# GuoYi0/alphaFive

Hardware: AMD Instinct MI355X
Metric: self-play moves/sec (11x11, 500 sims/move) (higher is better)
Workload: dtype f32 (fp16x2 split operands: 3 fp16 MFMA products per MAC, fp32 accumulate)

## Files before the change

alphafive_amd/csrc/af_engine.hip:

```cpp

#include <hip/hip_runtime.h>
#include <stdint.h>
#include <stdio.h>
#include <stdlib.h>
#include <string.h>

#include <type_traits>
#include <vector>

#include "af_engine.h"
#include "af_noise.h"

typedef unsigned long long u64;

enum { PH_IDLE = 0, PH_MOVE_START = 1, PH_SEARCH = 2, PH_MOVE_DONE = 3, PH_ERROR = 4, PH_DESCENT = 5  };
enum { CT_SIMS = 0, CT_SELECTS, CT_EXPANDS, CT_TERMINALS, CT_PLIES, CT_EPISODES, CT_LSUM, CT_LEXP,
       CT_GC, CT_GC_SCANNED, CT_YIELDS, CT_STALLS, CT_N };
enum { HIST_WORK = 0, HIST_TIME = 64, HIST_MAXTIME = 96, HIST_N = 97 };

struct EngineParams {
    int G, S, C, goal, sims, upper, training, mode, node_cap, max_ply, budget, budget_hard;
    uint32_t hash_mask;
    double init_temp, tau_decay, tau_decay_r, alpha, c_puct;
    float c_puct32;
// ... 3 lines not shown
    int32_t *action, *has_policy, *visits;
    float* policy;
    u64 *root, *leaf;
    double* tau;
    uint32_t *episode, *sel, *plyctr;
    int32_t *path_node, *path_cell;
    uint32_t* hash;
    u64* node_key;
    int32_t* node_sum;
    int32_t* free_idx;
    int32_t* edge_n;
    float *edge_w, *edge_p;
    int32_t* edge_c;
    double* edge_w64;
    int32_t w64;
    uint32_t *ep_seq, *ep_popped;
    int32_t* ep_len;
    float* ep_final;
    u64* rec_key;
    float* rec_policy;
    int32_t *rec_visits, *rec_last, *rec_action;
    u64* counters;
    u64* progress;
    u64* hist;
    u64* memo_key;
    float* memo_pv;
    float* memo_val;
    u64* memo_lock;
    u64* memo_stats;
    uint32_t memo_bucket_mask;
    int memo_max_stones;
    uint32_t memo_epoch;
    int memo_budget;
};
enum { MEMO_SERIAL = 0, MEMO_PROBES, MEMO_HITS, MEMO_INSERTS, MEMO_REPLACED, MEMO_N };

__device__ __forceinline__ uint32_t rfl32(uint32_t x) { return (uint32_t)__builtin_amdgcn_readfirstlane((int)x); }
__device__ __forceinline__ int rfli(int x) { return __builtin_amdgcn_readfirstlane(x); }
__device__ __forceinline__ u64 rfl64(u64 x) {
    return ((u64)rfl32((uint32_t)(x >> 32)) << 32) | (u64)rfl32((uint32_t)x);
}
__device__ __forceinline__ float rflf(float x) { return __int_as_float(rfli(__float_as_int(x))); }
template <int CTRL, int ROWS = 0xF>
__device__ __forceinline__ int dpp_i(int v) { return __builtin_amdgcn_update_dpp(v, v, CTRL, ROWS, 0xF, false); }
__device__ __forceinline__ int wave_max_i32(int v) {
    int o;
    o = dpp_i<0xB1>(v); v = o > v ? o : v;
    o = dpp_i<0x4E>(v); v = o > v ? o : v;
    o = dpp_i<0x141>(v); v = o > v ? o : v;
    o = dpp_i<0x140>(v); v = o > v ? o : v;
    o = dpp_i<0x142, 0xA>(v); v = o > v ? o : v;
    o = dpp_i<0x143, 0xC>(v); v = o > v ? o : v;
    return __builtin_amdgcn_readlane(v, 63);
}
__device__ __forceinline__ float wave_max_f32(float v) {
    float o;
    o = __int_as_float(dpp_i<0xB1>(__float_as_int(v))); v = o > v ? o : v;
    o = __int_as_float(dpp_i<0x4E>(__float_as_int(v))); v = o > v ? o : v;
    o = __int_as_float(dpp_i<0x141>(__float_as_int(v))); v = o > v ? o : v;
    o = __int_as_float(dpp_i<0x140>(__float_as_int(v))); v = o > v ? o : v;
    o = __int_as_float(dpp_i<0x142, 0xA>(__float_as_int(v))); v = o > v ? o : v;
    o = __int_as_float(dpp_i<0x143, 0xC>(__float_as_int(v))); v = o > v ? o : v;
    return __int_as_float(__builtin_amdgcn_readlane(__float_as_int(v), 63));
}


template <int CTRL>
// ... 340 lines not shown
        r.c[k] = R.ec[off];
        if constexpr (W64) r.w[k] = R.ew64[off]; else r.w[k] = R.ew[off];
        r.p[k] = R.ep[off];
    }
}

template <int KW, bool W64>
__device__ __forceinline__ void puct_scores(const EngineParams& P, int lane, const u64 (&legal)[KW], const int (&nn)[KW], const bool (&ff)[KW],
                                            const typename NodeRows<KW, W64>::wrow_t (&ww)[KW], const float (&pp)[KW],
                                            const double (&dd)[KW], bool is_root, int sum_n, float (&sc)[KW], float& mx) {
    const double sq = sqrt((double)(sum_n + 1));
    mx = -3.0e38f;
#pragma unroll
    for (int k = 0; k < KW; ++k) {
        const bool lg = (legal[k] >> lane) & 1ull;
        double q64;
        if (nn[k] == 0) q64 = 0.0;
        else if (!W64 && ff[k]) q64 = (double)((float)ww[k] / (float)nn[k]);
        else q64 = (double)ww[k] / (double)nn[k];
        double t;
        if (P.training) {
            double p_;
            if (is_root) p_ = (double)(0.75f * pp[k]) + 0.25 * dd[k];
            else p_ = (double)(0.9f * pp[k]) + 0.1 * dd[k];
            t = ((P.c_puct * p_) * sq) / (double)(1 + nn[k]);
        } else {
            t = ((double)(P.c_puct32 * pp[k]) * sq) / (double)(1 + nn[k]);
        }
        sc[k] = lg ? (float)(q64 + t) : -3.0e38f;
        mx = sc[k] > mx ? sc[k] : mx;
    }
}

template <int KW, bool W64, bool MEMO = false>
__global__ __launch_bounds__(64, AF_TICK_MIN_WAVES) void af_tick_kernel(EngineParams P, const float* __restrict__ policy_in,
                                                     const float* __restrict__ value_in, float* __restrict__ planes_out) {
    constexpr int CP = 64 * KW;
    __shared__ float s_pv[CP];
    __shared__ double s_cdf[CP];
    const int g = blockIdx.x;
    const int lane = threadIdx.x;
    const int C = P.C, NCAP = P.node_cap;
    if constexpr (MEMO) {
        if (g == 0 && lane == 0) atomicAdd(reinterpret_cast<unsigned long long*>(&P.memo_stats[MEMO_SERIAL]), 1ull);
    }

    int phase = rfli(P.phase[g]);
    if (phase == PH_IDLE || phase == PH_MOVE_DONE || phase == PH_ERROR) return;
    const u64 t_start = wall_clock64();
#ifdef AF_TICK_TIMING
    unsigned long long tk[13] = {0, 0, 0, 0, 0, 0, 0, 0, 0, 0, 0, 0, 0};
#endif
    TK_T(tk_entry);

    u64 root_m[KW], root_t[KW];
#pragma unroll
    for (int k = 0; k < KW; ++k) {
        root_m[k] = rfl64(P.root[(size_t)g * 2 * KW + k]);
        root_t[k] = rfl64(P.root[(size_t)g * 2 * KW + KW + k]);
    }
    int root_last = rfli(P.root_last[g]);
    int sims_left = rfli(P.sims_left[g]);
    int ply = rfli(P.ply[g]);
    int nodes = rfli(P.nodes[g]);
    int nfree = rfli(P.nfree[g]);
    double tau = P.tau[g];
    uint32_t episode = rfl32(P.episode[g]);
    uint32_t sel = rfl32(P.sel[g]);
    uint32_t plyctr = rfl32(P.plyctr[g]);
    const int random_a = rfli(P.random_a[g]);
    const uint32_t inv_s16 = (65536u + (uint32_t)P.S - 1u) / (uint32_t)P.S;
    const uint32_t k0 = P.k0, k1 = P.seed_hi + (P.first_game_id + (uint32_t)g);
    uint32_t ct[CT_N];
#pragma unroll
    for (int i = 0; i < CT_N; ++i) ct[i] = 0;
    int err = 0;

    GameRows R;
    game_rows<KW, W64>(P, g, NCAP, R);

    auto backup = [&](int depth, float v, int is_f32) {
        for (int d = lane; d < depth; d += 64) {
            const size_t off = (size_t)R.pnode[d] * CP + R.pcell[d];
            const float vv = ((depth - d) & 1) ? -v : v;
            const int32_t raw = R.en[off];
            if (W64) {
                R.en[off] = raw + 1;
                R.ew64[off] = R.ew64[off] + (double)vv;
            } else {
                R.en[off] = (raw + 1) | (is_f32 ? (int32_t)0x80000000 : 0);
                R.ew[off] = R.ew[off] + vv;
            }
        }
        __syncthreads();
    };

    TK_T(tk_loaded);
    TK_ACC(0, tk_entry, tk_loaded);
    u64 lm[KW], lt[KW];
    int c_depth = 0;
    uint32_t c_slot = 0;
    const float* c_pol = policy_in + (size_t)g * C;
// ... 221 lines not shown
            }
            if (ply >= P.max_ply) { err = AF_ERR_STATE; break; }
            const uint32_t seq = rfl32(P.ep_seq[g]);
            const size_t rslot = ((size_t)g * 2 + (seq & 1u)) * P.max_ply + ply;
            if (lane < 2 * KW) P.rec_key[rslot * 2 * KW + lane] = key_word<KW>(root_m, root_t, lane);
#pragma unroll
            for (int k = 0; k < KW; ++k) {
                const int c = lane + 64 * k;
                if (c < C) { P.rec_policy[rslot * C + c] = pol[k]; P.rec_visits[rslot * C + c] = nv[k] < 0 ? 0 : nv[k]; }
            }
            if (lane == 0) { P.rec_last[rslot] = root_last; P.rec_action[rslot] = action; }
            bb_step<KW>(root_m, root_t, action);
            root_last = action;
            ++ply;
            float fv;
            if (terminal_test<KW>(P, root_m, root_t, &fv)) {
                if (seq - rfl32(P.ep_popped[g]) >= 2u) { err = AF_ERR_EP_OVERRUN; break; }
                if (lane == 0) {
                    P.ep_len[(size_t)g * 2 + (seq & 1u)] = ply;
                    P.ep_final[(size_t)g * 2 + (seq & 1u)] = fv;
                    P.ep_seq[g] = seq + 1u;
                }
                ct[CT_EPISODES]++;
                if (lane == 0) atomicAdd(&P.progress[1], 1ull);
                for (uint32_t s_ = lane; s_ <= P.hash_mask; s_ += 64) R.slots[s_] = 0;
                __syncthreads();
                nodes = 0; nfree = 0;
#pragma unroll
                for (int k = 0; k < KW; ++k) { root_m[k] = 0; root_t[k] = 0; }
                root_last = -1;
                ply = 0;
                tau = P.init_temp;
                episode += 1; sel = 0; plyctr = 0;
            }
            phase = PH_MOVE_START;
            continue;
        }

        TK_T(tk_sim);
        TK_ACC(2, tk_iter, tk_sim);
        u64 cm[KW], ctb[KW];
        int last, depth;
        if (phase == PH_DESCENT) {
#pragma unroll
            for (int k = 0; k < KW; ++k) {
                cm[k] = rfl64(P.leaf[(size_t)g * 2 * KW + k]);
                ctb[k] = rfl64(P.leaf[(size_t)g * 2 * KW + KW + k]);
            }
            last = rfli(P.leaf_last[g]); depth = rfli(P.depth[g]);
            phase = PH_SEARCH;
        } else {
#pragma unroll
            for (int k = 0; k < KW; ++k) { cm[k] = root_m[k]; ctb[k] = root_t[k]; }
            last = root_last; depth = 0;
        }
        int hint = 0, pidx = -1, pcl = 0;
        typedef typename NodeRows<KW, W64>::wrow_t wrow_t;
        NodeRows<KW, W64> r;
        r.sum = 0;
        bool r_have = false;
        for (;;) {
            TK_T(tk_a);
            float tv;
            bool term;
            if (depth == 0)
                term = P.mode == AF_MODE_EXTERNAL ? (bool)terminal_test<KW, false>(P, cm, ctb, &tv) : false;
            else
                term = (depth > 0 && P.goal <= 8) ? (bool)terminal_through_last<KW>(P, cm, ctb, last, inv_s16, lane, &tv)
                                                                       : (bool)terminal_test<KW, true>(P, cm, ctb, &tv);
            if (term) {
                backup(depth, tv, 0);
                ct[CT_TERMINALS]++; ct[CT_SIMS]++;
                sims_left--;
                break;
            }
            uint32_t slot = 0xffffffffu;
            int idx;
            if (hint) {
                idx = hint - 1;
            } else {
                idx = tree_lookup<KW>(P, g, cm, ctb, lane, &slot);
                if (idx >= 0 && pidx >= 0 && lane == 0) R.ec[(size_t)pidx * CP + pcl] = idx + 1;
            }
            if (idx < 0) {
                if constexpr (MEMO) {
                    if (slot != 0xffffffffu && bb_count<KW>(cm) + bb_count<KW>(ctb) <= P.memo_max_stones) {
                        uint32_t unused;
                        const int me = memo_probe<KW>(P, memo_bucket<KW>(P, cm, ctb, last), cm, ctb, last, lane, &unused);
                        ++memo_probes;
                        if (me >= 0) {
                            ++memo_hits;
#pragma unroll
                            for (int k = 0; k < KW; ++k) { lm[k] = cm[k]; lt[k] = ctb[k]; }
// ... 3 lines not shown
                            have_eval = true;
                            break;
                        }
                    }
                }
                if (lane < 2 * KW) P.leaf[(size_t)g * 2 * KW + lane] = key_word<KW>(cm, ctb, lane);
                if (lane == 0) { P.depth[g] = depth; P.leaf_last[g] = last; P.leaf_slot[g] = (int32_t)slot; }
                float* out = planes_out + (size_t)g * 3 * C;
#pragma unroll
                for (int k = 0; k < KW; ++k) {
                    const int c = lane + 64 * k;
                    if (c < C) {
                        out[c] = ((cm[k] >> lane) & 1ull) ? 1.0f : 0.0f;
                        out[C + c] = ((ctb[k] >> lane) & 1ull) ? 1.0f : 0.0f;
                        out[2 * C + c] = c == last ? 1.0f : 0.0f;
                    }
                }
                status = AF_STATUS_NEED_EVAL;
                parked = true;
                break;
            }
            if (work >= P.budget_hard) {
                if (lane < 2 * KW) P.leaf[(size_t)g * 2 * KW + lane] = key_word<KW>(cm, ctb, lane);
                if (lane == 0) { P.depth[g] = depth; P.leaf_last[g] = last; }
                phase = PH_DESCENT; status = AF_STATUS_YIELD; parked = true; ct[CT_YIELDS]++;
                break;
            }
            TK_T(tk_b);
            TK_ACC(3, tk_a, tk_b);
            const bool is_root = depth == 0;
            u64 legal[KW];
#pragma unroll
            for (int k = 0; k < KW; ++k) legal[k] = ~(cm[k] | ctb[k]) & P.boardmask[k];
            if (!r_have) load_node_rows<KW, W64>(R, idx, lane, r);
            r_have = false;
            const int sum_n = rfli(r.sum) + 1;
            if (lane == 0) R.nsum[idx] = sum_n;
            const uint32_t sel_id = sel++;
            int nn[KW];
            float pp[KW];
            wrow_t ww[KW];
            bool ff[KW];
            int32_t cc[KW];
#pragma unroll
            for (int k = 0; k < KW; ++k) {
                nn[k] = r.raw[k] & 0x7fffffff;
                ff[k] = r.raw[k] < 0;
                cc[k] = r.c[k];
                ww[k] = r.w[k];
                pp[k] = r.p[k];
            }
            double dd[KW];
            if (P.training) {
#ifdef AF_TICK_TIMING
                int tk_myit = 0;
#endif
                {
                    const float a_ = (float)P.alpha, inv_a = 1.0f / a_, one_m_a = 1.0f - a_;
                    uint32_t todo = 0;
#pragma unroll
                    for (int k = 0; k < KW; ++k) { dd[k] = 0.0; todo |= ((legal[k] >> lane) & 1ull) ? (1u << k) : 0u; }
                    af_u32x4 rk[KW];
                    uint32_t pend = 0;
#pragma unroll
                    for (int k = 0; k < KW; ++k) {
                        rk[k] = af_philox4x32(sel_id, episode, (AF_STREAM_GAMMA << 24) | (uint32_t)(lane + 64 * k), 0u, k0, k1);
                        float X;
                        const int ok = af_gamma_round(a_, inv_a, one_m_a, rk[k].v[0], rk[k].v[1], &X);
                        const bool lg = (todo >> k) & 1u;
                        dd[k] = (lg && ok) ? (double)X : 0.0;
                        pend |= (lg && !ok) ? (1u << k) : 0u;
                        if (KW > 2 && (k & 1)) __builtin_amdgcn_sched_barrier(0);
                    }
#ifdef AF_TICK_TIMING
                    ++tk_myit;
#endif
                    todo = pend;
                    {
                    uint32_t it = 1;
                    af_u32x4 r = rk[0];
#pragma unroll
                    for (int q = 1; q < KW; ++q) if (!(todo & ((1u << q) - 1u))) r = rk[q];
                    while (todo) {
#ifdef AF_TICK_TIMING
                        ++tk_myit;
#endif
                        const int k = __builtin_ctz(todo);
                        if ((it & 1u) == 0u) r = af_philox4x32(sel_id, episode, (AF_STREAM_GAMMA << 24) | (uint32_t)(lane + 64 * k), it >> 1, k0, k1);
                        const uint32_t wu = (it & 1u) ? r.v[2] : r.v[0], wv = (it & 1u) ? r.v[3] : r.v[1];
                        float X;
                        const int ok = af_gamma_round(a_, inv_a, one_m_a, wu, wv, &X);
                        if (ok || it == 0xFFFFu) {
                            const double Xd = ok ? (double)X : 0.0;
#pragma unroll
                            for (int q = 0; q < KW; ++q) dd[q] = q == k ? Xd : dd[q];
                            todo &= todo - 1u;
                            it = 1;
#pragma unroll
                            for (int q = 1; q < KW; ++q) if (todo && !(todo & ((1u << q) - 1u))) r = rk[q];
                        } else {
                            ++it;
                        }
                    }
                    }
                }
#ifdef AF_TICK_TIMING
                tk[12] += (unsigned long long)wave_max_i32(tk_myit);
#endif
                TK_T(tk_n1);
                TK_ACC(8, tk_b, tk_n1);
                double acc = 0.0;
#pragma unroll
                for (int k = 0; k < KW; ++k) acc = k == 0 ? dd[0] : acc + dd[k];
                acc = wave_sum_f64_tree(acc);
                if (acc == 0.0) {
                    int cnt = 0;
#pragma unroll
                    for (int k = 0; k < KW; ++k) cnt += __popcll(legal[k]);
                    const double u = 1.0 / (double)cnt;
#pragma unroll
                    for (int k = 0; k < KW; ++k) dd[k] = ((legal[k] >> lane) & 1ull) ? u : 0.0;
                } else {
                    const double inv = 1.0 / acc;
#pragma unroll
                    for (int k = 0; k < KW; ++k) dd[k] = dd[k] * inv;
                }
                TK_T(tk_n1e);
                TK_ACC(9, tk_n1, tk_n1e);
            }
            TK_T(tk_n2);
            float sc[KW], mx;
            puct_scores<KW, W64>(P, lane, legal, nn, ff, ww, pp, dd, is_root, sum_n, sc, mx);
            TK_T(tk_n3);
            TK_ACC(10, tk_n2, tk_n3);
            int cell = -1;
            if (is_root && P.training) {
                u64 cand[KW];
#pragma unroll
                for (int k = 0; k < KW; ++k) cand[k] = __ballot(((legal[k] >> lane) & 1ull) && nn[k] == 0);
                int m = bb_count<KW>(cand);
                if (m == 0) {
#pragma unroll
                    for (int k = 0; k < KW; ++k) cand[k] = __ballot(((legal[k] >> lane) & 1ull) && nn[k] == 1);
                    m = bb_count<KW>(cand);
                }
                if (m > 0) cell = bb_select_wave<KW>(cand, (int)af_pick((uint32_t)m, sel_id, episode, AF_STREAM_PICK, k0, k1), lane);
            }
            if (cell < 0) {
                mx = wave_max_f32(mx);
                u64 cand[KW];
#pragma unroll
                for (int k = 0; k < KW; ++k) cand[k] = __ballot(((legal[k] >> lane) & 1ull) && sc[k] == mx);
                const int m = bb_count<KW>(cand);
                cell = bb_select_wave<KW>(cand, (int)af_pick((uint32_t)m, sel_id, episode, AF_STREAM_PICK, k0, k1), lane);
            }
            cell = rfli(cell);
            hint = 0;
#pragma unroll
            for (int k = 0; k < KW; ++k) { const int t_ = __builtin_amdgcn_readlane(cc[k], cell & 63); if ((cell >> 6) == k) hint = t_; }
            hint = rfli(hint);
            pidx = idx; pcl = cell;
            if (hint) {
                load_node_rows<KW, W64>(R, hint - 1, lane, r);
                r_have = true;
            }
            ++work;
            ct[CT_SELECTS]++;
            ct[CT_LSUM] += (uint32_t)bb_count<KW>(legal);
            if (lane == 0) { R.pnode[depth] = idx; R.pcell[depth] = cell; }
            ++depth;
            bb_step<KW>(cm, ctb, cell);
            last = cell;
            __syncthreads();
            TK_T(tk_c);
            TK_ACC(4, tk_b, tk_c);
            TK_ACC(11, tk_n3, tk_c);
#ifdef AF_TICK_TIMING
            tk[7] += 1;
#endif
        }
    }
    if (!MEMO || !have_eval) break;
  }
    TK_T(tk_parked);
    if constexpr (MEMO) {
        if (lane == 0 && memo_probes) {
            atomicAdd(reinterpret_cast<unsigned long long*>(&P.memo_stats[MEMO_PROBES]), (unsigned long long)memo_probes);
            if (memo_hits) atomicAdd(reinterpret_cast<unsigned long long*>(&P.memo_stats[MEMO_HITS]), (unsigned long long)memo_hits);
        }
    }

    if (err) { phase = PH_ERROR; status = err; }
    if (lane < 2 * KW) P.root[(size_t)g * 2 * KW + lane] = key_word<KW>(root_m, root_t, lane);
    if (lane == 0) {
        P.phase[g] = phase;
        P.pending[g] = status == AF_STATUS_NEED_EVAL ? 1 : 0;
        P.root_last[g] = root_last;
        P.sims_left[g] = sims_left;
        P.ply[g] = ply;
        P.nodes[g] = nodes;
        P.nfree[g] = nfree;
        P.tau[g] = tau;
        P.episode[g] = episode;
        P.sel[g] = sel;
        P.plyctr[g] = plyctr;
        P.status[g] = status;
        for (int i = 0; i < CT_N; ++i)
            if (ct[i]) atomicAdd(reinterpret_cast<unsigned long long*>(&P.counters[(size_t)g * CT_N + i]), (unsigned long long)ct[i]);
        const u64 dt = wall_clock64() - t_start;
        atomicAdd(&P.hist[HIST_WORK + (work < 63 ? work : 63)], 1ull);
        const u64 tb = dt / 800ull;
        atomicAdd(&P.hist[HIST_TIME + (tb < 31ull ? tb : 31ull)], 1ull);
        atomicMax(&P.hist[HIST_MAXTIME], dt);
    }
#ifdef AF_TICK_TIMING
    {
        TK_T(tk_end);
        tk[5] = tk_end - tk_parked;
        tk[6] = tk_end - tk_entry;
        if (lane == 0 && g < 8192) for (int q = 0; q < 13; ++q) g_tick_cycles[g][q] = tk[q];
    }
#endif
}

__global__ __launch_bounds__(1024) void af_pack_scan(EngineParams P, int max_eps, int max_plies, int32_t* __restrict__ out) {
    __shared__ int s_e[1024], s_p[1024];
    __shared__ int s_cut;
    const int t = threadIdx.x;
    int base_e = 0, base_p = 0;
    int32_t* meta = out + 4;
    int32_t* fin = out + 4 + (size_t)max_eps * 4;
    if (t == 0) s_cut = 0x7fffffff;
    __syncthreads();
    for (int g0 = 0; g0 < P.G; g0 += 1024) {
        const int g = g0 + t;
        int ne = 0, T0 = 0, T1 = 0;
        uint32_t pop = 0;
        if (g < P.G) {
            pop = P.ep_popped[g];
            ne = (int)(P.ep_seq[g] - pop);
            if (ne >= 1) T0 = P.ep_len[(size_t)g * 2 + (pop & 1u)];
            if (ne >= 2) T1 = P.ep_len[(size_t)g * 2 + ((pop + 1u) & 1u)];
        }
        s_e[t] = ne; s_p[t] = T0 + T1;
        __syncthreads();
        for (int off = 1; off < 1024; off <<= 1) {
// ... 354 lines not shown
    P.budget = AF_DEFAULT_TICK_BUDGET; P.budget_hard = AF_DEFAULT_TICK_BUDGET_HARD;
    if (const char* b = getenv("AF_TICK_BUDGET")) { const int v = atoi(b); if (v > 0) P.budget = v; }
    if (const char* b = getenv("AF_TICK_BUDGET_HARD")) { const int v = atoi(b); if (v > 0) P.budget_hard = v; }
    if (P.budget_hard < P.budget) P.budget_hard = P.budget;
    if (node_cap <= 0) node_cap = mode == AF_MODE_SELFPLAY ? 4 * P.sims + 64 : 32768;
    if (node_cap < P.sims + 8) node_cap = P.sims + 8;
    P.node_cap = node_cap;
    uint32_t hcap = 64;
    while (hcap < 2u * (uint32_t)node_cap) hcap <<= 1;
    P.hash_mask = hcap - 1;
    P.init_temp = cfg->init_temp; P.tau_decay = cfg->tau_decay_rate; P.tau_decay_r = cfg->tau_decay_rate_r;
    P.alpha = cfg->dirichlet_alpha; P.c_puct = cfg->c_puct; P.c_puct32 = (float)cfg->c_puct;
    P.k0 = af_key0(seed); P.seed_hi = (uint32_t)(seed >> 32); P.first_game_id = first_game_id;
    for (int c = 0; c < C; ++c) {
        P.boardmask[c >> 6] |= 1ull << (c & 63);
        if (c % S <= S - cfg->goal) P.colmask[c >> 6] |= 1ull << (c & 63);
    }
    const size_t G = num_games;
    int rc = AF_OK;
#define A(p, n) if (rc == AF_OK) rc = dalloc(e, &P.p, (n))
    A(phase, G); A(pending, G); A(sims_left, G); A(ply, G); A(root_last, G); A(nodes, G); A(nfree, G); A(depth, G);
    A(leaf_last, G); A(leaf_slot, G); A(status, G); A(random_a, G); A(action, G); A(has_policy, G);
    A(visits, G * CP); A(policy, G * CP); A(root, G * 2 * KW); A(leaf, G * 2 * KW); A(tau, G);
    A(episode, G); A(sel, G); A(plyctr, G); A(path_node, G * CP); A(path_cell, G * CP);
    A(hash, G * hcap); A(node_key, G * node_cap * 2 * KW); A(node_sum, G * node_cap); A(free_idx, G * node_cap);
    A(edge_n, G * node_cap * CP); A(edge_p, G * node_cap * CP); A(edge_c, G * node_cap * CP);
    if (value_f64) { A(edge_w64, G * node_cap * CP); A(edge_w, 64); } else { A(edge_w, G * node_cap * CP); A(edge_w64, 8); }
    A(ep_seq, G); A(ep_popped, G); A(counters, G * CT_N); A(progress, 2); A(hist, HIST_N);
    if (mode == AF_MODE_SELFPLAY) {
        const size_t R = G * 2 * P.max_ply;
        A(ep_len, G * 2); A(ep_final, G * 2); A(rec_key, R * 2 * KW); A(rec_policy, R * C); A(rec_visits, R * C);
        A(rec_last, R); A(rec_action, R);
    }
#undef A
    if (rc == AF_OK) rc = dalloc(e, &e->stamps, (size_t)AF_STAMP_SLOTS);
    if (rc != AF_OK) { af_engine_destroy(e); return rc; }
    std::vector<int32_t> ph(G, mode == AF_MODE_SELFPLAY ? PH_MOVE_START : PH_IDLE), rl(G, -1);
    std::vector<double> tau(G, cfg->init_temp);
    HIP_OK(hipMemcpy(P.phase, ph.data(), G * 4, hipMemcpyHostToDevice));
    HIP_OK(hipMemcpy(P.root_last, rl.data(), G * 4, hipMemcpyHostToDevice));
    HIP_OK(hipMemcpy(P.tau, tau.data(), G * 8, hipMemcpyHostToDevice));
    e->h_i32.resize(G); e->h_i32b.resize(G); e->h_ct.resize(G * CT_N);
    *out = e;
    return AF_OK;
}

void af_engine_destroy(af_engine* e) {
    if (!e) return;
    (void)hipSetDevice(e->device);
    for (void* p : e->allocs) (void)hipFree(p);
    if (e->stage_dev) (void)hipFree(e->stage_dev);
    delete e;
}

int32_t af_engine_num_games(const af_engine* e) { return e->P.G; }
int32_t af_engine_cells(const af_engine* e) { return e->P.C; }
int32_t af_engine_key_words(const af_engine* e) { return 2 * e->KW; }
int32_t af_engine_max_plies(const af_engine* e) { return e->P.max_ply; }

int af_engine_tick(af_engine* e, void* stream, const float* policy_dev, const float* value_dev, float* planes_dev) {
    if (!e || !planes_dev) return AF_ERR_ARG;
    hipStream_t st = (hipStream_t)stream;
    WITH_FLAG(e->memo, MEMO_, WITH_KW(e->KW, WITH_FLAG(e->P.w64, W64_,
        hipLaunchKernelGGL((af_tick_kernel<KW_, W64_, MEMO_>), dim3(e->P.G), dim3(64), 0, st, e->P, policy_dev, value_dev, planes_dev))));
    HIP_OK(hipGetLastError());
    return AF_OK;
}

int af_engine_memo_enable(af_engine* e, int32_t log2_buckets, int32_t max_stones) {
    if (!e || e->memo || log2_buckets < 4 || log2_buckets > 28 || max_stones < 0) return AF_ERR_ARG;
    HIP_OK(hipSetDevice(e->device));
    EngineParams& P = e->P;
    const size_t NE = (size_t)4 << log2_buckets, CP = 64 * (size_t)e->KW, MK = 4 * (size_t)e->KW;
    int rc = AF_OK;
    if (rc == AF_OK) rc = dalloc(e, &P.memo_key, NE * MK);
    if (rc == AF_OK) rc = dalloc(e, &P.memo_pv, NE * CP);
    if (rc == AF_OK) rc = dalloc(e, &P.memo_val, NE);
    if (rc == AF_OK) rc = dalloc(e, &P.memo_lock, NE);
    if (rc == AF_OK) rc = dalloc(e, &P.memo_stats, (size_t)MEMO_N);
    if (rc != AF_OK) return rc;
    P.memo_bucket_mask = (uint32_t)((1ull << log2_buckets) - 1ull);
    P.memo_max_stones = max_stones;
    P.memo_epoch = 1;
    P.memo_budget = P.budget < 6 ? P.budget : 6;
    if (const char* b = getenv("AF_MEMO_BUDGET")) { const int v = atoi(b); if (v > 0) { P.memo_budget = v; e->memo_budget_fixed = true; } }
    e->memo_entries = NE;
    e->memo = true;
    return AF_OK;
}

int af_engine_memo_insert(af_engine* e, void* stream, const float* policy_dev, const float* value_dev) {
    if (!e || !e->memo || !policy_dev || !value_dev) return AF_ERR_ARG;
    hipStream_t st = (hipStream_t)stream;
    WITH_KW(e->KW, hipLaunchKernelGGL((af_memo_insert_kernel<KW_>), dim3(e->P.G), dim3(64), 0, st, e->P, policy_dev, value_dev));
    HIP_OK(hipGetLastError());
    return AF_OK;
}
// ... 171 lines not shown
    if (!e || !out) return AF_ERR_ARG;
    hipStream_t st = (hipStream_t)stream;
    const int G = e->P.G;
    HIP_OK(hipMemcpyAsync(e->h_ct.data(), e->P.counters, (size_t)G * CT_N * 8, hipMemcpyDeviceToHost, st));
    HIP_OK(hipMemcpyAsync(e->h_i32.data(), e->P.nodes, (size_t)G * 4, hipMemcpyDeviceToHost, st));
    HIP_OK(hipMemcpyAsync(e->h_i32b.data(), e->P.nfree, (size_t)G * 4, hipMemcpyDeviceToHost, st));
    HIP_OK(hipStreamSynchronize(st));
    for (int i = 0; i < AF_NUM_COUNTERS; ++i) out[i] = 0;
    for (int g = 0; g < G; ++g) {
        for (int i = 0; i < 8; ++i) out[i] += e->h_ct[(size_t)g * CT_N + i];
        for (int i = 8; i < CT_N; ++i) out[i + 1] += e->h_ct[(size_t)g * CT_N + i];
        out[8] += (uint64_t)(e->h_i32[g] - e->h_i32b[g]);
    }
    return AF_OK;
}

int af_engine_tick_histogram(af_engine* e, void* stream, uint64_t* out, int32_t reset) {
    if (!e || !out) return AF_ERR_ARG;
    hipStream_t st = (hipStream_t)stream;
    HIP_OK(hipMemcpyAsync(out, e->P.hist, (size_t)HIST_N * 8, hipMemcpyDeviceToHost, st));
    if (reset) HIP_OK(hipMemsetAsync(e->P.hist, 0, (size_t)HIST_N * 8, st));
    HIP_OK(hipStreamSynchronize(st));
    return AF_OK;
}

int af_engine_set_tick_budget(af_engine* e, int32_t selects_per_launch) {
    if (!e || selects_per_launch < 1) return AF_ERR_ARG;
    e->P.budget = selects_per_launch;
    if (e->P.budget_hard < selects_per_launch) e->P.budget_hard = selects_per_launch;
    if (e->memo && !e->memo_budget_fixed) e->P.memo_budget = selects_per_launch < 6 ? selects_per_launch : 6;
    return AF_OK;
}

int af_engine_progress(af_engine* e, void* stream, uint64_t* out) {
    if (!e || !out) return AF_ERR_ARG;
    hipStream_t st = (hipStream_t)stream;
    HIP_OK(hipMemcpyAsync(out, e->P.progress, 16, hipMemcpyDeviceToHost, st));
    HIP_OK(hipStreamSynchronize(st));
    return AF_OK;
}

int af_engine_progress_async(af_engine* e, void* stream, uint64_t* out_pinned) {
    if (!e || !out_pinned) return AF_ERR_ARG;
    HIP_OK(hipMemcpyAsync(out_pinned, e->P.progress, 16, hipMemcpyDeviceToHost, (hipStream_t)stream));
    return AF_OK;
}

__global__ void af_stamp_kernel(unsigned long long* stamps, int slot) {
    if (threadIdx.x == 0) stamps[slot] = wall_clock64();
}

int af_engine_stamp(af_engine* e, void* stream, int32_t slot) {
    if (!e || slot < 0 || slot >= AF_STAMP_SLOTS) return AF_ERR_ARG;
    hipLaunchKernelGGL(af_stamp_kernel, dim3(1), dim3(64), 0, (hipStream_t)stream, e->stamps, (int)slot);
    HIP_OK(hipGetLastError());
    return AF_OK;
}

int af_engine_stamps_async(af_engine* e, void* stream, uint64_t* out_pinned) {
    if (!e || !out_pinned) return AF_ERR_ARG;
    HIP_OK(hipMemcpyAsync(out_pinned, e->stamps, AF_STAMP_SLOTS * 8, hipMemcpyDeviceToHost, (hipStream_t)stream));
    return AF_OK;
}

int af_match_create(af_engine* e0, af_engine* e1, af_match** out) {
    if (!e0 || !e1 || !out || e0 == e1) return AF_ERR_ARG;
// ... 238 lines not shown
```

alphafive_amd/engine.py:

```python
import ctypes as C
import os

import numpy as np

_PKG = os.path.dirname(os.path.abspath(__file__))
_LIBPATH = os.environ.get("AF_HIP_LIB") or os.path.join(_PKG, "_lib", "libaf_hip.so")

MODE_SELFPLAY, MODE_EXTERNAL = 0, 1
MODE_VALUE_F64 = 0x100
STATUS_IDLE, STATUS_NEED_EVAL, STATUS_MOVE_DONE, STATUS_YIELD = 0, 1, 2, 3
STAMP_SLOTS = 64
BLACK_WIN, WHITE_WIN, DRAW = 1, -1, 0

CFG_ATTRS = ("board_size", "goal", "simulation_per_step", "upper_simulation_per_step", "init_temp", "gamma",
             "tau_decay_rate", "tau_decay_rate_r", "dirichlet_alpha", "c_puct")


class AfConfig(C.Structure):
    _fields_ = [("board_size", C.c_int32), ("goal", C.c_int32), ("simulation_per_step", C.c_int32),
                ("upper_simulation_per_step", C.c_int32), ("init_temp", C.c_double), ("gamma", C.c_double),
                ("tau_decay_rate", C.c_double), ("tau_decay_rate_r", C.c_double), ("dirichlet_alpha", C.c_double),
                ("c_puct", C.c_double)]

    @classmethod
# ... 35 lines not shown
        L.af_engine_move_result.argtypes = [vp, C.c_int32, i32p, i32p, f32p, i32p, C.POINTER(C.c_double)]
        L.af_engine_set_training.argtypes = [vp, C.c_int32]
        L.af_engine_set_simulations.argtypes = [vp, C.c_int32, C.c_int32]
        L.af_engine_set_roots.argtypes = [vp, vp, C.c_int32, i32p, u64p, i32p, i32p, i32p]
        L.af_engine_move_results.argtypes = [vp, vp, C.c_int32, i32p, i32p, i32p, f32p, i32p, C.POINTER(C.c_double)]
        L.af_engine_pop_episodes.argtypes = [vp, vp, C.c_int32, i32p, f32p, u64p, f32p, i32p, i32p, i32p]
        L.af_engine_pack_ints.argtypes = [vp, C.c_int32, C.c_int32]
        L.af_engine_pack_ints.restype = C.c_int64
        L.af_engine_pack_episodes.argtypes = [vp, vp, C.c_int32, C.c_int32, vp]
        L.af_engine_counters.argtypes = [vp, vp, u64p]
        L.af_engine_tree_w64.argtypes = [vp, C.c_int32, C.c_int32, C.POINTER(C.c_double)]
        L.af_engine_set_tree_w64.argtypes = [vp, C.c_int32, C.c_int32, C.POINTER(C.c_double)]
        L.af_engine_progress.argtypes = [vp, vp, u64p]
        L.af_engine_progress_async.argtypes = [vp, vp, vp]
        L.af_engine_stamp.argtypes = [vp, vp, C.c_int32]
        L.af_engine_stamps_async.argtypes = [vp, vp, vp]
        L.af_engine_tick_histogram.argtypes = [vp, vp, u64p, C.c_int32]
        L.af_engine_set_tick_budget.argtypes = [vp, C.c_int32]
        L.af_engine_memo_enable.argtypes = [vp, C.c_int32, C.c_int32]
        L.af_engine_memo_insert.argtypes = [vp, vp, vp, vp]
        L.af_engine_memo_clear.argtypes = [vp, vp]
        L.af_engine_memo_stats.argtypes = [vp, vp, u64p]
        L.af_engine_memo_epoch.argtypes = [vp]
        L.af_engine_memo_epoch.restype = C.c_int64
        L.af_match_create.argtypes = [vp, vp, C.POINTER(vp)]
        L.af_match_destroy.argtypes = [vp]
        L.af_match_destroy.restype = None
        L.af_match_start.argtypes = [vp, vp, C.c_int32, C.c_int32]
        L.af_match_step.argtypes = [vp, vp]
        L.af_match_progress_async.argtypes = [vp, vp, vp]
        L.af_match_results.argtypes = [vp, vp, i32p, i32p, i32p]
        L.af_engine_tree_dump.argtypes = [vp, C.c_int32, C.c_int32, u64p, i32p, i32p, f32p, f32p, u8p]
        L.af_engine_load_tree.argtypes = [vp, C.c_int32, C.c_int32, u64p, i32p, i32p, f32p, f32p, u8p]
        L.af_state_to_key.argtypes = [C.c_char_p, C.c_int32, u64p]
        L.af_key_to_state.argtypes = [u64p, C.c_int32, C.c_char_p, C.c_int32]
        _lib = L
    return _lib


def _check(rc, what):
    if rc < 0:
        raise EngineError(f"{what}: {lib().af_strerror(rc).decode()} (code {rc})")
    return rc


def _p(a, ct):
    return a.ctypes.data_as(C.POINTER(ct))


def key_words(S):
    return 4 if S * S <= 128 else 8


def state_to_key(state, S):
    key = np.zeros(key_words(S), np.uint64)
    _check(lib().af_state_to_key(state.encode(), S, _p(key, C.c_uint64)), "af_state_to_key")
    return key


def key_to_state(key, S):
    key = np.ascontiguousarray(key, np.uint64)
    out = C.create_string_buffer(288)
    _check(lib().af_key_to_state(_p(key, C.c_uint64), S, out, 288), "af_key_to_state")
    return out.value.decode()


# ... 88 lines not shown

    def tick_histogram(self, stream=None, reset=False):
        out = np.zeros(97, np.uint64)
        _check(lib().af_engine_tick_histogram(self._h, stream, _p(out, C.c_uint64), int(reset)), "tick_histogram")
        return dict(selects=out[:64].astype(np.int64), wave_us=out[64:96].astype(np.int64),
                    max_wave_us=float(out[96]) * 0.01)

    def memo_enable(self, log2_buckets=18, max_stones=5):
        _check(lib().af_engine_memo_enable(self._h, int(log2_buckets), int(max_stones)), "af_engine_memo_enable")
        kw = self.KW2 // 2
        self.memo_bytes = (4 << int(log2_buckets)) * (32 * kw + 256 * kw + 12)
        self._params["memo"] = (int(log2_buckets), int(max_stones))
        self._params["memo_epoch"] = int(lib().af_engine_memo_epoch(self._h))

    @property
    def memo(self):
        return self._params.get("memo")

    def memo_insert(self, policy_ptr, value_ptr, stream=None):
        _check(lib().af_engine_memo_insert(self._h, stream, policy_ptr, value_ptr), "af_engine_memo_insert")

    def memo_clear(self, stream=None):
        _check(lib().af_engine_memo_clear(self._h, stream), "af_engine_memo_clear")
        self._params["memo_epoch"] = int(lib().af_engine_memo_epoch(self._h))

    def memo_stats(self, stream=None):
        out = np.zeros(6, np.uint64)
        _check(lib().af_engine_memo_stats(self._h, stream, _p(out, C.c_uint64)), "af_engine_memo_stats")
        return {k: int(v) for k, v in zip(("launches", "probes", "hits", "inserts", "replaced", "entries"), out)}

    def set_tick_budget(self, selects_per_launch):
        _check(lib().af_engine_set_tick_budget(self._h, int(selects_per_launch)), "af_engine_set_tick_budget")
        self._params["tick_budget"] = int(selects_per_launch)

    def progress(self, stream=None):
        out = np.zeros(2, np.uint64)
        _check(lib().af_engine_progress(self._h, stream, _p(out, C.c_uint64)), "af_engine_progress")
        return int(out[0]), int(out[1])

    def progress_async(self, out_ptr, stream=None):
        _check(lib().af_engine_progress_async(self._h, stream, out_ptr), "af_engine_progress_async")

    def stamp(self, slot, stream=None):
        _check(lib().af_engine_stamp(self._h, stream, int(slot)), "af_engine_stamp")

    def stamps_async(self, out_ptr, stream=None):
        _check(lib().af_engine_stamps_async(self._h, stream, out_ptr), "af_engine_stamps_async")

    def tree_dump(self, game):
        cnt = _check(lib().af_engine_tree_dump(self._h, game, 0, None, None, None, None, None, None), "tree_dump")
        keys = np.zeros((cnt, self.KW2), np.uint64)
        sum_n = np.zeros(cnt, np.int32)
        n = np.zeros((cnt, self.C), np.int32)
        w = np.zeros((cnt, self.C), np.float32)
        p = np.zeros((cnt, self.C), np.float32)
        f = np.zeros((cnt, self.C), np.uint8)
        if cnt:
            _check(lib().af_engine_tree_dump(self._h, game, cnt, _p(keys, C.c_uint64), _p(sum_n, C.c_int32),
                                             _p(n, C.c_int32), _p(w, C.c_float), _p(p, C.c_float), _p(f, C.c_uint8)),
                   "tree_dump")
            if self.value_f64:
                w = np.zeros((cnt, self.C), np.float64)
                _check(lib().af_engine_tree_w64(self._h, game, cnt, _p(w, C.c_double)), "af_engine_tree_w64")
        return dict(keys=keys, sum_n=sum_n, n=n, w=w, p=p, f32=f)

    def load_tree(self, game, dump):
# ... 291 lines not shown
```

include/af_engine.h:

```cpp
#ifndef AF_ENGINE_H
#define AF_ENGINE_H

#include <stdint.h>

#ifdef __cplusplus
extern "C" {
#endif

#define AF_ABI_VERSION 6

#define AF_MODE_SELFPLAY 0
#define AF_MODE_EXTERNAL 1
#define AF_MODE_VALUE_F64 0x100

#define AF_STATUS_IDLE      0
#define AF_STATUS_NEED_EVAL 1
#define AF_STATUS_MOVE_DONE 2
#define AF_STATUS_YIELD     3

#define AF_DEFAULT_TICK_BUDGET 8
#define AF_DEFAULT_TICK_BUDGET_HARD 12

#define AF_OK 0
#define AF_ERR_ARG        (-1)
// ... 34 lines not shown
int af_engine_set_root(af_engine* e, int32_t game, const uint64_t* key, int32_t last_cell, int32_t random_a,
                       int32_t reset_tree);
int af_engine_move_result(af_engine* e, int32_t game, int32_t* action_cell, int32_t* has_policy, float* policy,
                          int32_t* visits, double* tau);
int af_engine_set_training(af_engine* e, int32_t training);
int af_engine_set_simulations(af_engine* e, int32_t simulation_per_step, int32_t upper_simulation_per_step);

int af_engine_set_roots(af_engine* e, void* stream, int32_t n, const int32_t* games, const uint64_t* keys, const int32_t* last_cells,
                        const int32_t* random_a, const int32_t* reset_tree);
int af_engine_move_results(af_engine* e, void* stream, int32_t n, const int32_t* games, int32_t* action_cells, int32_t* has_policy,
                           float* policies, int32_t* visits, double* taus);

int64_t af_engine_pack_ints(const af_engine* e, int32_t max_episodes, int32_t max_plies);
int af_engine_pack_episodes(af_engine* e, void* stream, int32_t max_episodes, int32_t max_plies, int32_t* out);

int af_engine_pop_episodes(af_engine* e, void* stream, int32_t cap, int32_t* meta, float* final_value,
                           uint64_t* keys, float* policies, int32_t* visits, int32_t* lasts, int32_t* actions);

#define AF_NUM_COUNTERS 13
int af_engine_counters(af_engine* e, void* stream, uint64_t* out);

#define AF_MEMO_STATS 6
int af_engine_memo_enable(af_engine* e, int32_t log2_buckets, int32_t max_stones);
int af_engine_memo_insert(af_engine* e, void* stream, const float* policy_dev, const float* value_dev);
int af_engine_memo_clear(af_engine* e, void* stream);
int af_engine_memo_stats(af_engine* e, void* stream, uint64_t* out);
int64_t af_engine_memo_epoch(af_engine* e);

#define AF_HIST_WORDS 97
int af_engine_tick_histogram(af_engine* e, void* stream, uint64_t* out, int32_t reset);

int af_engine_set_tick_budget(af_engine* e, int32_t selects_per_launch);

int af_engine_progress(af_engine* e, void* stream, uint64_t* out);
int af_engine_progress_async(af_engine* e, void* stream, uint64_t* out_pinned);

#define AF_STAMP_SLOTS 64
int af_engine_stamp(af_engine* e, void* stream, int32_t slot);
int af_engine_stamps_async(af_engine* e, void* stream, uint64_t* out_pinned);

#define AF_MATCH_UNFINISHED (-1)
#define AF_MATCH_WIN0 0
#define AF_MATCH_WIN1 1
#define AF_MATCH_DRAW 2
typedef struct af_match af_match;
int af_match_create(af_engine* e0, af_engine* e1, af_match** out);
void af_match_destroy(af_match* m);
int af_match_start(af_match* m, void* stream, int32_t n_games, int32_t max_plies);
int af_match_step(af_match* m, void* stream);
int af_match_progress_async(af_match* m, void* stream, uint64_t* out_pinned);
int af_match_results(af_match* m, void* stream, int32_t* result, int32_t* lengths, int32_t* moves);

int af_engine_tree_dump(af_engine* e, int32_t game, int32_t cap, uint64_t* keys, int32_t* sum_n, int32_t* n,
                        float* w, float* p, uint8_t* f32);

int af_engine_load_tree(af_engine* e, int32_t game, int32_t count, const uint64_t* keys, const int32_t* sum_n,
                        const int32_t* n, const float* w, const float* p, const uint8_t* f32);

int af_engine_tree_w64(af_engine* e, int32_t game, int32_t cap, double* w);
int af_engine_set_tree_w64(af_engine* e, int32_t game, int32_t count, const double* w);

int af_state_to_key(const char* state, int32_t board_size, uint64_t* key);
int af_key_to_state(const uint64_t* key, int32_t board_size, char* out, int32_t cap);

const char* af_strerror(int code);
int af_abi_version(void);
// ... 6 lines not shown
```

Measured before the change: 6035.

## Precompute Dirichlet gamma noise rows in extra blocks via per-game ring

Launches a second set of blocks alongside the tick kernel that precompute the gamma noise rows for upcoming selections into a per-game ring buffer tagged by episode and selection id. The select loop loads the matching row with the node rows and uses it when the tag matches, falling back to inline rejection sampling otherwise. This moves the costly per-select gamma sampling off the critical path of the search waves, at the cost of doubling the block count, extra global memory traffic and a fill window that can miss after episode resets.

```diff
diff --git a/alphafive_amd/csrc/af_engine.hip b/alphafive_amd/csrc/af_engine.hip
--- a/alphafive_amd/csrc/af_engine.hip
+++ b/alphafive_amd/csrc/af_engine.hip
@@ -59,7 +59,13 @@
     int memo_max_stones;
     uint32_t memo_epoch;
     int memo_budget;
+    float* ring;
+    uint32_t* ring_tag;
+    uint32_t* ring_fill;
+    u64* ring_stats;
+    int ring_n;
 };
+enum { RING_MISS = 0, RING_COLD, RING_STATS_N };
 enum { MEMO_SERIAL = 0, MEMO_PROBES, MEMO_HITS, MEMO_INSERTS, MEMO_REPLACED, MEMO_N };
 
 __device__ __forceinline__ uint32_t rfl32(uint32_t x) { return (uint32_t)__builtin_amdgcn_readfirstlane((int)x); }
@@ -466,14 +472,76 @@
     }
 }
 
+template <int KW>
+struct NoiseRow {
+    float v[KW];
+    uint32_t ep, id;
+};
+template <int KW>
+__device__ __forceinline__ void load_noise_row(const EngineParams& P, int g, uint32_t slot, int lane, NoiseRow<KW>& nr) {
+    constexpr int CP = 64 * KW;
+    const size_t ro = (size_t)g * P.ring_n + slot;
+    nr.ep = P.ring_tag[2 * ro];
+    nr.id = P.ring_tag[2 * ro + 1];
+#pragma unroll
+    for (int k = 0; k < KW; ++k) nr.v[k] = P.ring[ro * CP + lane + 64 * k];
+}
+
+template <int KW>
+__device__ __forceinline__ void noise_fill(const EngineParams& P, int g, int lane) {
+    constexpr int CP = 64 * KW;
+    const uint32_t N = (uint32_t)P.ring_n, hard = (uint32_t)P.budget_hard;
+    const uint32_t E = rfl32(P.episode[g]), s = rfl32(P.sel[g]);
+    const uint32_t end = rfl32(P.ring_fill[2 * g]), ep = rfl32(P.ring_fill[2 * g + 1]);
+    uint32_t lo = s + hard;
+    const uint32_t hi = s + N;
+    if (ep == E && end - s <= N && end - s > hard) lo = end;
+    if (hard >= N) lo = hi;
+    const uint32_t rows = hi - lo;
+    if (rows == 0) return;
+    const uint32_t k0 = P.k0, k1 = P.seed_hi + (P.first_game_id + (uint32_t)g);
+    const float a_ = (float)P.alpha, inv_a = 1.0f / a_, one_m_a = 1.0f - a_;
+    float* ring = P.ring + (size_t)g * N * CP;
+    uint32_t* tags = P.ring_tag + (size_t)g * N * 2;
+    const uint32_t slot0 = lo % N;
+    const uint32_t total = rows * KW;
+    uint32_t j = 0, it = 0;
+    af_u32x4 r;
+    r.v[0] = r.v[1] = r.v[2] = r.v[3] = 0;
+    while (j < total) {
+        const uint32_t row = j / KW, k = j % KW, cell = (uint32_t)lane + 64u * k;
+        if (cell >= (uint32_t)P.C) { ++j; continue; }
+        if ((it & 1u) == 0u) r = af_philox4x32(lo + row, E, (AF_STREAM_GAMMA << 24) | cell, it >> 1, k0, k1);
+        const uint32_t wu = (it & 1u) ? r.v[2] : r.v[0], wv = (it & 1u) ? r.v[3] : r.v[1];
+        float X;
+        const int ok = af_gamma_round(a_, inv_a, one_m_a, wu, wv, &X);
+        if (ok || it == 0xFFFFu) {
+            uint32_t slot = slot0 + row;
+            slot = slot >= N ? slot - N : slot;
+            ring[(size_t)slot * CP + cell] = ok ? X : 0.0f;
+            ++j; it = 0;
+        } else {
+            ++it;
+        }
+    }
+    for (uint32_t row = (uint32_t)lane; row < rows; row += 64u) {
+        uint32_t slot = slot0 + row;
+        slot = slot >= N ? slot - N : slot;
+        tags[2 * slot] = E;
+        tags[2 * slot + 1] = lo + row;
+    }
+    if (lane == 0) { P.ring_fill[2 * g] = hi; P.ring_fill[2 * g + 1] = E; }
+}
+
 template <int KW, bool W64, bool MEMO = false>
 __global__ __launch_bounds__(64, AF_TICK_MIN_WAVES) void af_tick_kernel(EngineParams P, const float* __restrict__ policy_in,
                                                      const float* __restrict__ value_in, float* __restrict__ planes_out) {
     constexpr int CP = 64 * KW;
     __shared__ float s_pv[CP];
     __shared__ double s_cdf[CP];
+    const int lane = threadIdx.x;
+    if ((int)blockIdx.x >= P.G) { noise_fill<KW>(P, (int)blockIdx.x - P.G, lane); return; }
     const int g = blockIdx.x;
-    const int lane = threadIdx.x;
     const int C = P.C, NCAP = P.node_cap;
     if constexpr (MEMO) {
         if (g == 0 && lane == 0) atomicAdd(reinterpret_cast<unsigned long long*>(&P.memo_stats[MEMO_SERIAL]), 1ull);
@@ -502,6 +570,9 @@
     uint32_t episode = rfl32(P.episode[g]);
     uint32_t sel = rfl32(P.sel[g]);
     uint32_t plyctr = rfl32(P.plyctr[g]);
+    const bool ring_on = P.ring != nullptr;
+    uint32_t ring_slot = ring_on ? sel % (uint32_t)P.ring_n : 0u;
+    uint32_t ring_miss = 0, ring_cold = 0;
     const int random_a = rfli(P.random_a[g]);
     const uint32_t inv_s16 = (65536u + (uint32_t)P.S - 1u) / (uint32_t)P.S;
     const uint32_t k0 = P.k0, k1 = P.seed_hi + (P.first_game_id + (uint32_t)g);
@@ -789,6 +860,7 @@
                 ply = 0;
                 tau = P.init_temp;
                 episode += 1; sel = 0; plyctr = 0;
+                ring_slot = 0;
             }
             phase = PH_MOVE_START;
             continue;
@@ -816,6 +888,10 @@
         NodeRows<KW, W64> r;
         r.sum = 0;
         bool r_have = false;
+        NoiseRow<KW> nz;
+        nz.ep = 0; nz.id = 0;
+#pragma unroll
+        for (int k = 0; k < KW; ++k) nz.v[k] = 0.0f;
         for (;;) {
             TK_T(tk_a);
             float tv;
@@ -885,11 +961,15 @@
             u64 legal[KW];
 #pragma unroll
             for (int k = 0; k < KW; ++k) legal[k] = ~(cm[k] | ctb[k]) & P.boardmask[k];
-            if (!r_have) load_node_rows<KW, W64>(R, idx, lane, r);
+            if (!r_have) {
+                load_node_rows<KW, W64>(R, idx, lane, r);
+                if (P.training && ring_on) load_noise_row<KW>(P, g, ring_slot, lane, nz);
+            }
             r_have = false;
             const int sum_n = rfli(r.sum) + 1;
             if (lane == 0) R.nsum[idx] = sum_n;
             const uint32_t sel_id = sel++;
+            ring_slot = ring_slot + 1u == (uint32_t)P.ring_n ? 0u : ring_slot + 1u;
             int nn[KW];
             float pp[KW];
             wrow_t ww[KW];
@@ -908,7 +988,19 @@
 #ifdef AF_TICK_TIMING
                 int tk_myit = 0;
 #endif
-                {
+                const bool ring_hit = ring_on && rfl32(nz.ep) == episode && rfl32(nz.id) == sel_id;
+                if (ring_hit) {
+#pragma unroll
+                    for (int k = 0; k < KW; ++k) dd[k] = ((legal[k] >> lane) & 1ull) ? (double)nz.v[k] : 0.0;
+                } else {
+                    if (ring_on) { if (sel_id >= 2u * (uint32_t)P.budget_hard) ++ring_miss; else ++ring_cold; }
+#ifdef AF_NOISE_PRICE
+#pragma unroll
+                    for (int k = 0; k < KW; ++k) {
+                        const size_t o_ = (size_t)(sel_id & 7u) * CP + lane + 64 * k;
+                        dd[k] = ((legal[k] >> lane) & 1ull) ? (double)(R.ep[o_] + R.ep[o_ + (size_t)8 * CP]) + 0.5 : 0.0;
+                    }
+#else
                     const float a_ = (float)P.alpha, inv_a = 1.0f / a_, one_m_a = 1.0f - a_;
                     uint32_t todo = 0;
 #pragma unroll
@@ -956,6 +1048,7 @@
                         }
                     }
                     }
+#endif
                 }
 #ifdef AF_TICK_TIMING
                 tk[12] += (unsigned long long)wave_max_i32(tk_myit);
@@ -1015,6 +1108,7 @@
             pidx = idx; pcl = cell;
             if (hint) {
                 load_node_rows<KW, W64>(R, hint - 1, lane, r);
+                if (P.training && ring_on) load_noise_row<KW>(P, g, ring_slot, lane, nz);
                 r_have = true;
             }
             ++work;
@@ -1065,6 +1159,8 @@
         const u64 tb = dt / 800ull;
         atomicAdd(&P.hist[HIST_TIME + (tb < 31ull ? tb : 31ull)], 1ull);
         atomicMax(&P.hist[HIST_MAXTIME], dt);
+        if (ring_miss) atomicAdd(reinterpret_cast<unsigned long long*>(&P.ring_stats[RING_MISS]), (unsigned long long)ring_miss);
+        if (ring_cold) atomicAdd(reinterpret_cast<unsigned long long*>(&P.ring_stats[RING_COLD]), (unsigned long long)ring_cold);
     }
 #ifdef AF_TICK_TIMING
     {
@@ -1485,6 +1581,12 @@
         A(ep_len, G * 2); A(ep_final, G * 2); A(rec_key, R * 2 * KW); A(rec_policy, R * C); A(rec_visits, R * C);
         A(rec_last, R); A(rec_action, R);
     }
+    const char* ring_env = getenv("AF_NOISE_RING");
+    if (P.training && !(ring_env && atoi(ring_env) == 0)) {
+        P.ring_n = 3 * P.budget_hard > AF_NOISE_RING_ROWS ? 3 * P.budget_hard : AF_NOISE_RING_ROWS;
+        A(ring, G * P.ring_n * CP); A(ring_tag, G * P.ring_n * 2); A(ring_fill, G * 2); A(ring_stats, (size_t)RING_STATS_N);
+        if (rc == AF_OK && hipMemset(P.ring_tag, 0xFF, G * P.ring_n * 2 * sizeof(uint32_t)) != hipSuccess) rc = AF_ERR_HIP;
+    }
 #undef A
     if (rc == AF_OK) rc = dalloc(e, &e->stamps, (size_t)AF_STAMP_SLOTS);
     if (rc != AF_OK) { af_engine_destroy(e); return rc; }
@@ -1514,8 +1616,9 @@
 int af_engine_tick(af_engine* e, void* stream, const float* policy_dev, const float* value_dev, float* planes_dev) {
     if (!e || !planes_dev) return AF_ERR_ARG;
     hipStream_t st = (hipStream_t)stream;
+    const int blocks = (e->P.ring && e->P.training) ? 2 * e->P.G : e->P.G;
     WITH_FLAG(e->memo, MEMO_, WITH_KW(e->KW, WITH_FLAG(e->P.w64, W64_,
-        hipLaunchKernelGGL((af_tick_kernel<KW_, W64_, MEMO_>), dim3(e->P.G), dim3(64), 0, st, e->P, policy_dev, value_dev, planes_dev))));
+        hipLaunchKernelGGL((af_tick_kernel<KW_, W64_, MEMO_>), dim3(blocks), dim3(64), 0, st, e->P, policy_dev, value_dev, planes_dev))));
     HIP_OK(hipGetLastError());
     return AF_OK;
 }
@@ -1753,6 +1856,45 @@
     return AF_OK;
 }
 
+int32_t af_engine_noise_ring_rows(const af_engine* e) { return (e && e->P.ring) ? e->P.ring_n : 0; }
+
+int af_engine_noise_row(af_engine* e, int32_t game, uint32_t sel_id, float* out, uint32_t tag[2]) {
+    if (!e || !e->P.ring || game < 0 || game >= e->P.G || !out || !tag) return AF_ERR_ARG;
+    const EngineParams& P = e->P;
+    const size_t ro = (size_t)game * P.ring_n + sel_id % (uint32_t)P.ring_n, CP = 64 * (size_t)e->KW;
+    HIP_OK(hipDeviceSynchronize());
+    HIP_OK(hipMemcpy(out, P.ring + ro * CP, (size_t)P.C * 4, hipMemcpyDeviceToHost));
+    HIP_OK(hipMemcpy(tag, P.ring_tag + 2 * ro, 8, hipMemcpyDeviceToHost));
+    return AF_OK;
+}
+
+int af_engine_noise_state(af_engine* e, int32_t game, uint32_t out[4]) {
+    if (!e || !e->P.ring || game < 0 || game >= e->P.G || !out) return AF_ERR_ARG;
+    HIP_OK(hipDeviceSynchronize());
+    HIP_OK(hipMemcpy(out, e->P.episode + game, 4, hipMemcpyDeviceToHost));
+    HIP_OK(hipMemcpy(out + 1, e->P.sel + game, 4, hipMemcpyDeviceToHost));
+    HIP_OK(hipMemcpy(out + 2, e->P.ring_fill + 2 * (size_t)game, 8, hipMemcpyDeviceToHost));
+    return AF_OK;
+}
+
+int af_engine_noise_stats(af_engine* e, void* stream, uint64_t* out) {
+    if (!e || !out) return AF_ERR_ARG;
+    out[0] = out[1] = 0;
+    if (!e->P.ring) return AF_OK;
+    hipStream_t st = (hipStream_t)stream;
+    HIP_OK(hipMemcpyAsync(out, e->P.ring_stats, (size_t)RING_STATS_N * 8, hipMemcpyDeviceToHost, st));
+    HIP_OK(hipStreamSynchronize(st));
+    return AF_OK;
+}
+
+float af_noise_gamma_ref(double alpha, uint64_t seed, uint32_t game_id, uint32_t episode, uint32_t sel_id, uint32_t cell) {
+    return (float)af_gamma_lt1(alpha, sel_id, episode, cell, af_key0(seed), af_key1(seed, game_id));
+}
+
+void af_noise_gamma_ref_row(double alpha, uint64_t seed, uint32_t game_id, uint32_t episode, uint32_t sel_id, int32_t cells, float* out) {
+    for (int32_t c = 0; c < cells; ++c) out[c] = af_noise_gamma_ref(alpha, seed, game_id, episode, sel_id, (uint32_t)c);
+}
+
 int af_engine_progress(af_engine* e, void* stream, uint64_t* out) {
     if (!e || !out) return AF_ERR_ARG;
     hipStream_t st = (hipStream_t)stream;
diff --git a/alphafive_amd/engine.py b/alphafive_amd/engine.py
--- a/alphafive_amd/engine.py
+++ b/alphafive_amd/engine.py
@@ -91,6 +91,17 @@
         L.af_match_results.argtypes = [vp, vp, i32p, i32p, i32p]
         L.af_engine_tree_dump.argtypes = [vp, C.c_int32, C.c_int32, u64p, i32p, i32p, f32p, f32p, u8p]
         L.af_engine_load_tree.argtypes = [vp, C.c_int32, C.c_int32, u64p, i32p, i32p, f32p, f32p, u8p]
+        if hasattr(L, "af_engine_noise_ring_rows"):
+            u32p = C.POINTER(C.c_uint32)
+            L.af_engine_noise_ring_rows.argtypes = [vp]
+            L.af_engine_noise_ring_rows.restype = C.c_int32
+            L.af_engine_noise_row.argtypes = [vp, C.c_int32, C.c_uint32, f32p, u32p]
+            L.af_engine_noise_state.argtypes = [vp, C.c_int32, u32p]
+            L.af_engine_noise_stats.argtypes = [vp, vp, u64p]
+            L.af_noise_gamma_ref.argtypes = [C.c_double, C.c_uint64, C.c_uint32, C.c_uint32, C.c_uint32, C.c_uint32]
+            L.af_noise_gamma_ref.restype = C.c_float
+            L.af_noise_gamma_ref_row.argtypes = [C.c_double, C.c_uint64, C.c_uint32, C.c_uint32, C.c_uint32, C.c_int32, f32p]
+            L.af_noise_gamma_ref_row.restype = None
         L.af_state_to_key.argtypes = [C.c_char_p, C.c_int32, u64p]
         L.af_key_to_state.argtypes = [u64p, C.c_int32, C.c_char_p, C.c_int32]
         _lib = L
@@ -245,6 +256,25 @@
     def set_tick_budget(self, selects_per_launch):
         _check(lib().af_engine_set_tick_budget(self._h, int(selects_per_launch)), "af_engine_set_tick_budget")
         self._params["tick_budget"] = int(selects_per_launch)
+
+    @property
+    def noise_ring_rows(self):
+        return int(lib().af_engine_noise_ring_rows(self._h))
+
+    def noise_row(self, game, sel_id):
+        out, tag = np.zeros(self.C, np.float32), np.zeros(2, np.uint32)
+        _check(lib().af_engine_noise_row(self._h, int(game), int(sel_id), _p(out, C.c_float), _p(tag, C.c_uint32)), "af_engine_noise_row")
+        return out, (int(tag[0]), int(tag[1]))
+
+    def noise_state(self, game):
+        out = np.zeros(4, np.uint32)
+        _check(lib().af_engine_noise_state(self._h, int(game), _p(out, C.c_uint32)), "af_engine_noise_state")
+        return dict(zip(("episode", "sel", "ring_end", "ring_episode"), (int(v) for v in out)))
+
+    def noise_stats(self, stream=None):
+        out = np.zeros(2, np.uint64)
+        _check(lib().af_engine_noise_stats(self._h, stream, _p(out, C.c_uint64)), "af_engine_noise_stats")
+        return {"misses": int(out[0]), "cold": int(out[1])}
 
     def progress(self, stream=None):
         out = np.zeros(2, np.uint64)
diff --git a/include/af_engine.h b/include/af_engine.h
--- a/include/af_engine.h
+++ b/include/af_engine.h
@@ -90,6 +90,14 @@
 
 int af_engine_set_tick_budget(af_engine* e, int32_t selects_per_launch);
 
+#define AF_NOISE_RING_ROWS 36
+int32_t af_engine_noise_ring_rows(const af_engine* e);
+int af_engine_noise_row(af_engine* e, int32_t game, uint32_t sel_id, float* out, uint32_t tag[2]);
+int af_engine_noise_state(af_engine* e, int32_t game, uint32_t out[4]);
+int af_engine_noise_stats(af_engine* e, void* stream, uint64_t* out);
+float af_noise_gamma_ref(double alpha, uint64_t seed, uint32_t game_id, uint32_t episode, uint32_t sel_id, uint32_t cell);
+void af_noise_gamma_ref_row(double alpha, uint64_t seed, uint32_t game_id, uint32_t episode, uint32_t sel_id, int32_t cells, float* out);
+
 int af_engine_progress(af_engine* e, void* stream, uint64_t* out);
 int af_engine_progress_async(af_engine* e, void* stream, uint64_t* out_pinned);
 
```

Measured after the change: 6035, median of 2. Within noise of the previous version (+0.0%).
